# MaartenGr/ReinLife

Hardware: AMD Instinct MI355X
Metric: agent-steps/sec (env.step + policy fwd), 30x30 grid, 100 agents (higher is better)
Workload: dtype f32-grade policy via block-scaled 2 x f16 split on v_mfma_f32_32x32x16_f16 (f32 accumulate) / int32+u8 world state / f64 rewards

## Files before the change

reinlife_amd/csrc/rl_policy_dev.h:

```cpp
#pragma once
#include "rl_common.h"

namespace {

typedef float f32x16 __attribute__((ext_vector_type(16)));
typedef float f32x4 __attribute__((ext_vector_type(4)));
typedef float f32x4u __attribute__((ext_vector_type(4), aligned(4)));
typedef float f32x2 __attribute__((ext_vector_type(2)));
typedef _Float16 f16x8 __attribute__((ext_vector_type(8)));
typedef const float __attribute__((address_space(1))) gfloat;
typedef const f32x4 __attribute__((address_space(1))) gf32x4;

constexpr int kInChunks = 10;
constexpr int kPlanes = 2;
constexpr int kScaleExp = 10;

__host__ __device__ constexpr int64_t frag_floats(int chunks, int tout) { return (int64_t)chunks * tout * kPlanes * 64 * 4; }
__host__ __device__ constexpr int64_t in_layer_floats(int tout) { return frag_floats(kInChunks, tout) + (int64_t)tout * 64; }
__host__ __device__ constexpr int64_t hid_layer_floats(int tin, int tout) { return frag_floats(2 * tin, tout) + (int64_t)tout * 64; }
__host__ __device__ constexpr int64_t head_consts_off(int tin) { return frag_floats(2 * tin, 1); }
__host__ __device__ constexpr int64_t head_floats(int tin, int nout) { return head_consts_off(tin) + 16; }

struct Layout {
    int64_t l1, l2a, l2b, ha, hb, total;
// ... 337 lines not shown
        split8(x, sc0, B1[c][0], B1[c][1]);
    }
    f32x16 acc[4];
    RL_PMARK1(2);
    k_loop_reg4<kInChunks>(w, B1, acc);
    RL_PMARK1(3);
    w.start(packed + L.l2a, lane, 0);
    f32x4 B2[8][kPlanes], B3[8][kPlanes];
    float un1, un2;
    layer_out_to_B(acc, packed + L.l1 + frag_floats(kInChunks, 4), h, un0, B2, un1);
    RL_PMARK1(4);
    k_loop_reg4<8>(w, B2, acc);
    RL_PMARK1(5);
    layer_out_to_B(acc, packed + L.l2a + frag_floats(8, 4), h, un1, B3, un2);
    float adv[4], val[4];
    RL_PMARK1(6);
    head_reg<4>(packed + L.ha, B3, un2, lane, adv);
    RL_PMARK1(7);
    w.start(packed + L.l2b, lane, 0);
    k_loop_reg4<8>(w, B2, acc);
    RL_PMARK1(8);
    layer_out_to_B(acc, packed + L.l2b + frag_floats(8, 4), h, un1, B3, un2);
    head_reg<4>(packed + L.hb, B3, un2, lane, val);
    RL_PMARK1(9);
    const f32x4 ba = ((gf32x4*)(packed + L.ha + head_consts_off(4) + 8))[h];
    tile1_finish<KIND>(io, lane, adv, val[0] + packed[L.hb + head_consts_off(4) + 8], draw, ba);
}

constexpr int kStageUnits = 512;
constexpr int kStages = 10 + 8 + 2 + 8 + 2;
constexpr int kDenseTiles = 4;

constexpr int kTileConstFloats = 3 * 256 + 2 * 16;

template <int NS, int D, int STEPS = 2 * NS, int TOUT = 4>
struct WRingH {
    f32x4 a[D][2][kPlanes];
    gf32x4* p;
#ifdef RL_ABL_WH
    static __host__ __device__ constexpr int off(int i) { return 0; }
#else
    static __host__ __device__ constexpr int off(int i) { return ((i % NS) * TOUT + 2 * (i / NS)) * kPlanes * 64; }
#endif
    __device__ inline void start(gfloat* __restrict__ pw, int lane)
    {
        static_assert(D < NS, "ring deeper than a pass");
        p = (gf32x4*)pw + lane;
#pragma unroll
        for (int d = 0; d < D; ++d)
#pragma unroll
            for (int t = 0; t < 2; ++t)
#pragma unroll
                for (int pl = 0; pl < kPlanes; ++pl) a[d][t][pl] = p[off(d) + (t * kPlanes + pl) * 64];
        p += off(D);
        asm volatile("" : "+v"(p));
    }
    __device__ inline void take(int i, f32x4 (&ac)[2][kPlanes])
    {
        const int cur = i % D;
#pragma unroll
        for (int t = 0; t < 2; ++t)
#pragma unroll
            for (int pl = 0; pl < kPlanes; ++pl) ac[t][pl] = a[cur][t][pl];
        if (i + D < STEPS) {
#pragma unroll
            for (int t = 0; t < 2; ++t)
// ... 126 lines not shown
    f32x16 a0, a1, a2;
#pragma unroll
    for (int r = 0; r < 16; ++r) { a0[r] = 0.0f; a1[r] = 0.0f; a2[r] = 0.0f; }
    f32x4 B[NCH][kPlanes];
#pragma unroll
    for (int k = 0; k < 3; ++k) split_slice<3>(k, [&](int e) { return raw(0, e); }, sc, B[0][0], B[0][1]);
#pragma unroll
    for (int s = 0; s < NCH; ++s) {
        f32x4 ac[1][kPlanes];
        w.template next<NCH>(s, ac);
        a0 = mfma16(ac[0][0], B[s][1], a0);
        if (s + 1 < NCH) split_slice<3>(0, [&](int e) { return raw(s + 1, e); }, sc, B[(s + 1) % NCH][0], B[(s + 1) % NCH][1]);
        __builtin_amdgcn_sched_barrier(0);
        a1 = mfma16(ac[0][0], B[s][0], a1);
        if (s + 1 < NCH) split_slice<3>(1, [&](int e) { return raw(s + 1, e); }, sc, B[(s + 1) % NCH][0], B[(s + 1) % NCH][1]);
        __builtin_amdgcn_sched_barrier(0);
        a2 = mfma16(ac[0][1], B[s][0], a2);
        if (s + 1 < NCH) split_slice<3>(2, [&](int e) { return raw(s + 1, e); }, sc, B[(s + 1) % NCH][0], B[(s + 1) % NCH][1]);
        __builtin_amdgcn_sched_barrier(0);
    }
#pragma unroll
    for (int r = 0; r < 4; ++r) out[r] = ((a0[r] + a1[r]) + a2[r]) * (un4[r] * row_un);
}

struct PairLds {
    float* pmax;
    f32x4* ex;
    float* val;
};
struct Tile1Part {
    float head[4];
    rl_u4 draw;
};
template <int KIND, bool COHERENT, bool PAIR = false, int XM = 0>
__device__ inline void policy_tile1s(const TileIO& io, int lane, int role = 0, const PairLds* pair_lds = nullptr, Tile1Part* part = nullptr)
{
    static_assert(KIND == RL_D3QN || KIND == RL_PERD3QN, "one-wave tile: dueling kinds");
    extern __shared__ __attribute__((aligned(16))) char rl_dyn_lds[];
    constexpr int D = 3;
    const int h = lane >> 5;
    const Layout L = layout_of(KIND);
    gfloat* __restrict__ packed = io.packed;
    const float* const consts = (const float*)(rl_dyn_lds + io.c_lds_off) + 32 * h;
    const float* const hconsts = (const float*)(rl_dyn_lds + io.c_lds_off) + 768;
    RL_PMARK1(1);
    WRingH<kInChunks, D, PAIR ? kInChunks : 2 * kInChunks> w1;
    w1.start(packed + L.l1 + (PAIR ? role * (2 * kPlanes * 64 * 4) : 0), lane);
    f32x4 X[kInChunks][2];
    {
        const int64_t rbase = io.row * RL_OBS_DIM;
        if (io.x_lds_off >= 0) {
            const float* xr = (const float*)(rl_dyn_lds + io.x_lds_off);
#pragma unroll
            for (int c = 0; c < kInChunks; ++c)
#pragma unroll
                for (int q = 0; q < 2; ++q) {
                    if (c == kInChunks - 1 && h == 1) X[c][q] = f32x4{xr[149], xr[150], xr[151], xr[152]};
                    else X[c][q] = *(const f32x4*)(xr + 16 * c + 8 * h + 4 * q);
                }
        } else
#pragma unroll
        for (int c = 0; c < kInChunks; ++c)
#pragma unroll
            for (int q = 0; q < 2; ++q) {
                const int k0 = (c == kInChunks - 1 && h == 1) ? 149 : 16 * c + 8 * h + 4 * q;
                if (COHERENT) {
                    const __amdgpu_buffer_rsrc_t rsrc = __builtin_amdgcn_make_buffer_rsrc((void*)io.obs, 0, 0x7fffffff, 0x00027000);
                    X[c][q] = __builtin_bit_cast(f32x4, __builtin_amdgcn_raw_buffer_load_b128(rsrc, (int)((rbase + k0) * 4), 0, 16 ));
                } else
                    X[c][q] = *(const f32x4u*)(io.obs + rbase + k0);
// ... 15 lines not shown
            }
        float m = fmaxf(fmaxf(m4[0], m4[1]), fmaxf(m4[2], m4[3]));
        m = fmaxf(m, __shfl_xor(m, 32));
        row_scale(m, sc0, un0);
    }
    f32x4 B1[kInChunks][kPlanes];
    auto xraw = [&](int c, int e) { return X[c][e >> 2][e & 3]; };
    f32x16 F[4];
    EpiStream ep;
    if constexpr (XM >= 1) {
        auto x0 = [&](int e) { return xraw(0, e); };
        in_split_slot<XM, 0, 0>(x0, sc0, B1[0][0], B1[0][1]); in_split_slot<XM, 0, 1>(x0, sc0, B1[0][0], B1[0][1]);
        in_split_slot<XM, 0, 2>(x0, sc0, B1[0][0], B1[0][1]); in_split_slot<XM, 0, 3>(x0, sc0, B1[0][0], B1[0][1]);
        RL_PMARK1(2);
        k_pass_inx<0, XM>(w1, B1, F[0], F[1], [&](auto st, auto k, auto) {
            constexpr int c = decltype(st)::value + 1;
            if constexpr (c < kInChunks) in_split_slot<XM, c, decltype(k)::value>([&](int e) { return xraw(c, e); }, sc0, B1[c][0], B1[c][1]);
        });
    } else {
#pragma unroll
        for (int k = 0; k < 6; ++k) split_slice<6>(k, [&](int e) { return xraw(0, e); }, sc0, B1[0][0], B1[0][1]);
        RL_PMARK1(2);
        k_pass<kInChunks, 0>(w1, B1, F[0], F[1], [&](int slot) {
            const int c = slot / 6 + 1;
            if (c < kInChunks) split_slice<6>(slot % 6, [&](int e) { return xraw(c, e); }, sc0, B1[c][0], B1[c][1]);
        });
    }
    float mrow = 0.0f;
    const int64_t l2 = (PAIR && role) ? L.l2b : L.l2a, hd = (PAIR && role) ? L.hb : L.ha;
    WRingH<8, D> w2;
    f32x4 B2[8][kPlanes];
    float sc1, un1;
    auto fraw = [&](int c, int e) { return F[c >> 1][8 * (c & 1) + e]; };
    if (PAIR) {
        w2.start(packed + l2, lane);
        ep.c = consts + role * 128;
        ep.fetch(0, 0);
#pragma unroll
        for (int e = 0; e < 32; ++e) ep.step(0, e, F[0], F[1], un0, mrow);
        mrow = fmaxf(mrow, __shfl_xor(mrow, 32));
        pair_lds->pmax[role * 64 + lane] = mrow;
        lds_barrier();
        mrow = fmaxf(mrow, pair_lds->pmax[(role ^ 1) * 64 + lane]);
        row_scale(mrow, sc1, un1);
#pragma unroll
        for (int c = 0; c < 4; ++c) {
            f32x4 hi, lo;
#pragma unroll
            for (int k = 0; k < 6; ++k) split_slice<6>(k, [&](int e) { return fraw(c, e); }, sc1, hi, lo);
            pair_lds->ex[((4 * role + c) * kPlanes + 0) * 64 + lane] = hi;
            pair_lds->ex[((4 * role + c) * kPlanes + 1) * 64 + lane] = lo;
        }
        lds_barrier();
#pragma unroll
        for (int c = 0; c < 8; ++c)
#pragma unroll
            for (int pl = 0; pl < kPlanes; ++pl) B2[c][pl] = pair_lds->ex[(c * kPlanes + pl) * 64 + lane];
    } else {
        ep.c = consts;
        if constexpr (XM >= 1)
            k_pass_inx<1, XM>(w1, B1, F[2], F[3], [&](auto, auto, auto sl) {
                constexpr int slot = decltype(sl)::value;
                if constexpr (slot == 0) ep.fetch(0, 0);
                if constexpr (slot >= 2 && slot < 34) ep.step(0, slot - 2, F[0], F[1], un0, mrow);
            });
        else
        k_pass<kInChunks, 1>(w1, B1, F[2], F[3], [&](int slot) {
            if (slot == 0) ep.fetch(0, 0);
            if (slot >= 2 && slot < 34) ep.step(0, slot - 2, F[0], F[1], un0, mrow);
        });
        RL_PMARK1(3);
        w2.start(packed + l2, lane);
        ep.fetch(2, 0);
#pragma unroll
        for (int e = 0; e < 32; ++e) ep.step(2, e, F[2], F[3], un0, mrow);
        mrow = fmaxf(mrow, __shfl_xor(mrow, 32));
        row_scale(mrow, sc1, un1);
#pragma unroll
        for (int k = 0; k < 6; ++k) split_slice<6>(k, [&](int e) { return fraw(0, e); }, sc1, B2[0][0], B2[0][1]);
    }
    RL_PMARK1(4);
    f32x16 A[4];
    k_pass<8, 0>(w2, B2, A[0], A[1], [&](int slot) {
        const int c = slot / 6 + 1;
        if (!PAIR && c < 8) split_slice<6>(slot % 6, [&](int e) { return fraw(c, e); }, sc1, B2[c][0], B2[c][1]);
    });
    mrow = 0.0f;
    ep.c = consts + ((PAIR && role) ? 512 : 256);
    k_pass<8, 1>(w2, B2, A[2], A[3], [&](int slot) {
        if (slot == 0) ep.fetch(0, 0);
        if (slot >= 2 && slot < 34) ep.step(0, slot - 2, A[0], A[1], un1, mrow);
    });
    RL_PMARK1(5);
    WRing<1, 1, 1, D> wh;
    wh.start(packed + hd, lane, 0);
    ep.fetch(2, 0);
#pragma unroll
    for (int e = 0; e < 32; ++e) ep.step(2, e, A[2], A[3], un1, mrow);
    mrow = fmaxf(mrow, __shfl_xor(mrow, 32));
    float sc2, un2;
    row_scale(mrow, sc2, un2);
    auto araw = [&](int c, int e) { return A[c >> 1][8 * (c & 1) + e]; };
    float adv[4], val[4];
    RL_PMARK1(6);
    if (PAIR) {
        head_stream<D>(wh, *(const f32x4*)(hconsts + ((PAIR && role) ? 16 : 0) + 4 * h), araw, sc2, un2, adv);
        if (role) { if (h == 0) pair_lds->val[lane] = adv[0] + hconsts[16 + 8]; }
        else {
#pragma unroll
            for (int r = 0; r < 4; ++r) part->head[r] = adv[r];
            part->draw = draw;
        }
        RL_PMARK1(9);
        return;
    }
    head_stream<D>(wh, *(const f32x4*)(hconsts + 4 * h), araw, sc2, un2, adv);
    WRingH<8, D> w3;
    w3.start(packed + L.l2b, lane);
    RL_PMARK1(7);
    k_pass<8, 0>(w3, B2, A[0], A[1], [&](int) {});
    mrow = 0.0f;
    ep.c = consts + 512;
    k_pass<8, 1>(w3, B2, A[2], A[3], [&](int slot) {
        if (slot == 0) ep.fetch(0, 0);
        if (slot >= 2 && slot < 34) ep.step(0, slot - 2, A[0], A[1], un1, mrow);
    });
    RL_PMARK1(8);
    wh.start(packed + L.hb, lane, 0);
    ep.fetch(2, 0);
#pragma unroll
    for (int e = 0; e < 32; ++e) ep.step(2, e, A[2], A[3], un1, mrow);
    mrow = fmaxf(mrow, __shfl_xor(mrow, 32));
    row_scale(mrow, sc2, un2);
    head_stream<D>(wh, *(const f32x4*)(hconsts + 16 + 4 * h), araw, sc2, un2, val);
    RL_PMARK1(9);
    tile1_finish<KIND>(io, lane, adv, val[0] + hconsts[16 + 8], draw, *(const f32x4*)(hconsts + 8 + 4 * h));
}


// ... 809 lines not shown
```

reinlife_amd/csrc/rl_run.hip:

```cpp
#include <mutex>
#include "rl_world_dev.h"
#ifndef RL_XM_DUELING_KERNEL
#define RL_XM_DUELING_KERNEL 0
#endif
#if RL_XM_DUELING_KERNEL != 0 && !defined(RL_XM_SELF_GENERATED_STATES_ONLY)
#error "RL_XM_DUELING_KERNEL != 0 is valid for self-generated states only: add -DRL_XM_SELF_GENERATED_STATES_ONLY to an A/B build that knows"
#endif
#ifndef RL_XM_ALL_DUELING_TILE
#define RL_XM_ALL_DUELING_TILE RL_XM_ALL_KERNEL
#endif
#ifndef RL_XM_ALL_KERNEL
#define RL_XM_ALL_KERNEL 2
#endif

#ifdef RL_TUNING
#if !(defined(RL_RUN_UNIT) && RL_RUN_UNIT == 1)
static int g_run_debug = 0;
extern "C" __attribute__((visibility("default"))) void rl_debug_set_run_mask(int mask) { g_run_debug = mask; }
extern "C" __attribute__((visibility("default"))) int rl_debug_get_run_mask(void) { return g_run_debug; }
#endif
#define RL_RUN_DBG(ka) (*(const int __attribute__((address_space(4)))*)&(ka)->ra.debug)
#else
#define RL_RUN_DBG(ka) 0
#endif

namespace {

#include "rl_policy_dev.h"

constexpr int kRunMaxBrains = 8;
constexpr int kKindAll = 4;
__host__ __device__ constexpr int kind_widest(int KIND) { return KIND == kKindAll ? RL_PPO : KIND; }

#ifndef RL_RUN_COHERENT
#define RL_RUN_COHERENT true
#endif
struct RunArgs {
    const float* packed[kRunMaxBrains];
    float eps[kRunMaxBrains];
    int kind[kRunMaxBrains];
    float* obs[2];
    int first;
    int n_ticks;
    int8_t* actions;
    const float* eps_sched;
    int eps_inline_on;
    float eps_inline[RL_EPS_INLINE_MAX];
    int trk_skip;
    int capture;
    float* policy_out;
    rl_replay rp[kRunMaxBrains];
    int debug;
};

struct PolSmem {
    short* prow;
    int* bstart;
    int* bcnt;
    int* tstart;
    short* trow;
    int* tbrain;
    int* meta;
    float* pairv;
    float* cconst;
    float* xmirror;
    int xrows;
    int xbytes;
    double* trk_scr;
    TrkLds trk;
    int* wtask;
    int* texoff;
    int* bkind;
    int* oflags;
};
constexpr int kMaxTiles = 32;
constexpr int kPairFloats = 32 + 2 * 64;
constexpr int kPairExBytes = 8 * kPlanes * 64 * 16;
constexpr int kPairFloatsAll = kPairValFloats + 2 * 64;
template <int KIND> __host__ __device__ constexpr int run_const_floats() { return KIND == kKindAll ? kTileConstMax : kTileConstFloats; }
template <int KIND> __host__ __device__ constexpr int run_pair_floats() { return KIND == kKindAll ? kPairFloatsAll : kPairFloats; }
template <int KIND>
__host__ __device__ inline size_t carve_policy(PolSmem& ps, char* base, size_t o, int cap, size_t mirror_budget = 0, int n_cbrains = 0,
                                               int pair_floats = run_pair_floats<KIND>(),
                                               size_t min_region = 0)
{
    o = align16(o);
    ps.xmirror = nullptr; ps.xrows = 0; ps.xbytes = 0;
    const size_t tail = 10 * (size_t)cap + 5120 + sizeof(float) * 4 * (size_t)pair_floats + sizeof(float) * run_const_floats<KIND>() * (size_t)n_cbrains;
    if (mirror_budget > o + tail) {
        const size_t rows = (mirror_budget - o - tail) / (sizeof(float) * kXStride);
        ps.xrows = (int)(rows < (size_t)cap ? rows : (size_t)cap);
        if (ps.xrows >= 32) {
            size_t bytes = sizeof(float) * kXStride * (size_t)ps.xrows;
            if (bytes < min_region && o + tail + min_region <= mirror_budget) bytes = min_region;
            ps.xmirror = (float*)(base + o); ps.xbytes = (int)bytes; o = align16(o + bytes);
        } else ps.xrows = 0;
    }
    ps.prow = (short*)(base + o); o = align16(o + sizeof(short) * (size_t)cap);
    ps.bstart = (int*)(base + o); o = align16(o + sizeof(int) * 64);
    ps.bcnt = (int*)(base + o); o = align16(o + sizeof(int) * 64);
    ps.tstart = (int*)(base + o); o = align16(o + sizeof(int) * 64);
    ps.trow = (short*)(base + o); o = align16(o + sizeof(short) * kMaxTiles * 32);
    ps.tbrain = (int*)(base + o); o = align16(o + sizeof(int) * kMaxTiles);
    ps.meta = (int*)(base + o); o = align16(o + sizeof(int) * 16);
    ps.cconst = nullptr;
    if (n_cbrains > 0) { ps.cconst = (float*)(base + o); o = align16(o + sizeof(float) * run_const_floats<KIND>() * (size_t)n_cbrains); }
    ps.pairv = nullptr;
    if (n_cbrains > 0) { ps.pairv = (float*)(base + o); o = align16(o + sizeof(float) * 4 * (size_t)pair_floats); }
    ps.wtask = (int*)(base + o); o = align16(o + sizeof(int) * 8);
    ps.texoff = (int*)(base + o); o = align16(o + sizeof(int) * 4);
    ps.bkind = (int*)(base + o); o = align16(o + sizeof(int) * kRunMaxBrains);
    if (KIND == kKindAll) { ps.oflags = (int*)(base + o); o = align16(o + sizeof(int) * 4); }
// ... 216 lines not shown
        io.prof = (p.prof && (int)blockIdx.x == p.prof_world && wave == 0) ? p.prof : nullptr;
        if (io.prof && lane == 0) { io.prof[100] = t_entry; io.prof[110] = (long long)clock64(); }
#endif
    };
    if constexpr (T == 1024) {
        const int q = __builtin_amdgcn_readfirstlane(wave >> 2), slot = wave & 3;
        for (int t0 = 0; t0 < ntiles; t0 += 4) {
            const int lane = rl_lane_fresh(), j = lane & 31;
            const int ti = t0 + slot;
            const bool have = ti < ntiles;
            TileIO io;
            Tile1Part part;
            QuadLds ql;
            ql.pmax = ps.pairv + kQuadFloats * slot; ql.val = ql.pmax + 3 * 32 * 4;
            ql.ex = (f32x4*)((char*)ps.xmirror + (size_t)kQuadExBytes * slot);
#ifdef RL_PHASE_PROFILE
            ql.prof = (p.prof && (int)blockIdx.x == p.prof_world && slot == 0) ? p.prof : nullptr;
#endif
            if (have) {
                tile_io(ti, io, j);
                if (ntiles > 4) io.x_lds_off = -1;
                policy_quad<KIND, RL_RUN_COHERENT>(io, lane, q, &ql, &part);
            } else {
#pragma unroll
                for (int i = 0; i < kQuadBarriers; ++i) lds_barrier();
            }
            lds_barrier();
            if (have && q == 0) tile1_finish<KIND>(io, lane, part.head, ql.val[j], part.draw, *(const f32x4*)((const float*)(smem_base + io.c_lds_off) + 768 + 8 + 4 * (lane >> 5)));
        }
    } else
    if (T == 512 && ps.pairv != nullptr && ntiles <= 4 && (size_t)ps.xrows * kXStride * sizeof(float) >= 4 * (size_t)kPairExBytes) {
        const int role = __builtin_amdgcn_readfirstlane(wave >> 2), slot = wave & 3;
        const bool have = slot < ntiles;
        TileIO io;
        Tile1Part part;
        PairLds pl;
        pl.val = ps.pairv + kPairFloats * slot; pl.pmax = pl.val + 32;
        pl.ex = (f32x4*)((char*)ps.xmirror + (size_t)kPairExBytes * slot);
        if (have) {
            tile_io(slot, io, j);
            policy_tile1s<KIND, RL_RUN_COHERENT, true, RL_XM_DUELING_KERNEL>(io, lane, role, &pl, &part);
        } else { lds_barrier(); lds_barrier(); }
#ifdef RL_PHASE_PROFILE
        if (p.prof && (int)blockIdx.x == p.prof_world && lane == 0) p.prof[116 + wave] = (long long)clock64();
#endif
        lds_barrier();
        if (have && role == 0) {
            const int fl = rl_lane_fresh();
            tile1_finish<KIND>(io, fl, part.head, pl.val[fl & 31], part.draw, *(const f32x4*)((const float*)(smem_base + io.c_lds_off) + 768 + 8 + 4 * (fl >> 5)));
        }
    } else
    for (int ti = wave; ti < ntiles; ti += T / 64) {
        TileIO io;
        tile_io(ti, io, j);
        if (T == 512) policy_tile1s<KIND, RL_RUN_COHERENT, false, RL_XM_DUELING_KERNEL>(io, lane);
        else policy_tile1<KIND, RL_RUN_COHERENT, true>(io, lane);
    }
#ifdef RL_PHASE_PROFILE
    if (p.prof && (int)blockIdx.x == p.prof_world && tid == 0) p.prof[111] = (long long)clock64();
#endif
    lds_barrier();
#ifdef RL_PHASE_PROFILE
    if (p.prof && (int)blockIdx.x == p.prof_world && tid == 0) p.prof[112] = (long long)clock64();
#endif
}

#ifndef RL_XM_COLD_CALL
#define RL_XM_COLD_CALL 0
#endif
#ifndef RL_XM_LIKELY
#define RL_XM_LIKELY 1
#endif
#if RL_XM_LIKELY
#define RL_XM_EXPECT(x) __builtin_expect_with_probability(!!(x), 1, 0.9)
#else
#define RL_XM_EXPECT(x) (x)
#endif
__device__ __attribute__((noinline, cold)) Tile1Part run_tile_general(TileIO io, PairLds pl, int role, int kind)
{
    Tile1Part part;
    const int lane = rl_lane_fresh();
    if (kind == RL_DQN) policy_pair2<RL_DQN, RL_RUN_COHERENT>(io, lane, role, &pl, &part);
    else if (kind == RL_PPO) policy_pair2<RL_PPO, RL_RUN_COHERENT>(io, lane, role, &pl, &part);
    else policy_tile1s<RL_PERD3QN, RL_RUN_COHERENT, true>(io, lane, role, &pl, &part);
    return part;
}

template <int T, int TRAIN>
__device__ __forceinline__ void run_policy_all(const KParams& p, Smem& s, PolSmem& ps, RunParamsC* ka, int w, int n, const float* obs_rows, char* smem_base, int wave)
{
    static_assert(T == 512, "kKindAll: 512-thread workgroups");
    typedef const int __attribute__((address_space(4))) cint;
    const int lane = rl_lane_fresh(), j = lane & 31;
#ifdef RL_PHASE_PROFILE
    if (p.prof && (int)blockIdx.x == p.prof_world && wave == 0 && lane == 0) p.prof[100] = (long long)clock64();
#endif
    const int ntiles = __builtin_amdgcn_readfirstlane(ps.meta[0]);
    const bool mirrored = ps.xmirror != nullptr && __builtin_amdgcn_readfirstlane(ps.meta[4]) != 0;
    const bool fallback = __builtin_amdgcn_readfirstlane(ps.meta[5]) != 0;
    constexpr int xneed = RL_XM_ALL_KERNEL == 2 ? (RL_XF_SCALE | RL_XF_INT_HEALTH) : RL_XF_SCALE;
#ifdef RL_XM_ASSUME_ALWAYS
    const bool rows_known = true;
#else
    const bool rows_known = RL_XM_ALL_KERNEL != 0 && (__builtin_amdgcn_readfirstlane(ps.oflags[0]) & xneed) == xneed;
#endif
    auto tile_io = [&](int ti, TileIO& io, bool from_mirror, int task) {
        const int b = task >= 0 ? ((task >> 12) & 255) : __builtin_amdgcn_readfirstlane(ps.tbrain[ti]);
        const int e = (unsigned short)ps.trow[ti * 32 + j], k = e & 0x7fff;
        io.packed = (gfloat*)((const float* const __attribute__((address_space(4)))*)ka->ra.packed)[b];
        io.obs = obs_rows;
        io.row = (int64_t)w * p.cap + k;
        io.valid = !(e & 0x8000);
        io.eps = run_eps<TRAIN>(ka, b, p.n_brains, ps);
        io.out = TRAIN == 2 ? *(float* const __attribute__((address_space(4)))*)&ka->ra.policy_out : nullptr;
        io.actions = *(int8_t* const __attribute__((address_space(4)))*)&ka->ra.actions;
        io.seed = p.seed;
        io.key_world = (uint32_t)(p.world_base + w); io.key_tick = (uint32_t)s.scal[S_TICK]; io.key_epoch = (uint32_t)s.scal[S_EPOCH];
        io.key_index = (uint32_t)k;
        io.lds_actions_off = (int)((char*)s.action - smem_base); io.lds_slot = k;
        io.x_lds_off = (from_mirror && mirrored && k < ps.xrows) ? (int)((char*)(ps.xmirror + k * kXStride) - smem_base) : -1;
        io.c_lds_off = (int)((char*)(ps.cconst + kTileConstMax * b) - smem_base);
#ifdef RL_PHASE_PROFILE
        io.prof = (p.prof && (int)blockIdx.x == p.prof_world && wave == ((p.ablate >> 20) & 7)) ? p.prof : nullptr;
#endif
        return task >= 0 ? ((task >> 20) & 7) : ((cint*)ka->ra.kind)[b];
    };
    auto pair_round = [&](bool have, int ti, int role, int slot, int ex_off, bool from_mirror, int task) {
        TileIO io;
        Tile1Part part;
        PairLds pl;
        int kind = -1;
        if (have) {
            kind = __builtin_amdgcn_readfirstlane(tile_io(ti, io, from_mirror, task));
            pl.val = ps.pairv + kPairFloatsAll * slot; pl.pmax = pl.val + kPairValFloats;
            pl.ex = (f32x4*)((char*)ps.xmirror + ex_off);
            const bool plain = kind == RL_DQN || kind == RL_PPO;
            if (!plain && RL_XM_ALL_DUELING_TILE == 0) policy_tile1s<RL_PERD3QN, RL_RUN_COHERENT, true>(io, lane, role, &pl, &part);
            else if (RL_XM_EXPECT(rows_known)) {
                if (kind == RL_DQN) policy_pair2<RL_DQN, RL_RUN_COHERENT, RL_XM_ALL_KERNEL>(io, lane, role, &pl, &part);
                else if (kind == RL_PPO) policy_pair2<RL_PPO, RL_RUN_COHERENT, RL_XM_ALL_KERNEL>(io, lane, role, &pl, &part);
                else policy_tile1s<RL_PERD3QN, RL_RUN_COHERENT, true, RL_XM_ALL_DUELING_TILE>(io, lane, role, &pl, &part);
            } else if (RL_XM_COLD_CALL) part = run_tile_general(io, pl, role, kind);
            else {
                if (kind == RL_DQN) policy_pair2<RL_DQN, RL_RUN_COHERENT>(io, lane, role, &pl, &part);
                else if (kind == RL_PPO) policy_pair2<RL_PPO, RL_RUN_COHERENT>(io, lane, role, &pl, &part);
                else policy_tile1s<RL_PERD3QN, RL_RUN_COHERENT, true>(io, lane, role, &pl, &part);
            }
        } else { lds_barrier(); lds_barrier(); }
        lds_barrier();
        if (have && role == 0) {
            const int fl = rl_lane_fresh();
            if (kind == RL_DQN) pair_finish<RL_DQN>(io, fl, part, &pl);
            else if (kind == RL_PPO) pair_finish<RL_PPO>(io, fl, part, &pl);
            else tile1_finish<RL_PERD3QN>(io, fl, part.head, pl.val[fl & 31], part.draw, *(const f32x4*)((const float*)(smem_base + io.c_lds_off) + 768 + 8 + 4 * (fl >> 5)));
        }
    };
    const int pr = __builtin_amdgcn_readfirstlane(ps.meta[6]);
    const int task = __builtin_amdgcn_readfirstlane(ps.wtask[wave]);
    const int n_rounds = fallback ? (ntiles + pr - 1) / pr : 1;
    for (int r = 0; r < n_rounds; ++r) {
        const int slot = fallback ? (wave & 3) : (task & 255);
        const int ti = fallback ? r * pr + slot : slot;
        const bool have = fallback ? (slot < pr && ti < ntiles) : task >= 0;
        const int role = __builtin_amdgcn_readfirstlane(fallback ? (wave >> 2) : ((task >> 8) & 1));
        const int ex_off = fallback ? slot * pair_ex_bytes(RL_PPO) : (have ? ps.texoff[slot] : 0);
        pair_round(have, ti, role, slot, ex_off, !fallback, fallback ? -1 : task);
        if (fallback) lds_barrier();
    }
#ifdef RL_PHASE_PROFILE
    if (p.prof && (int)blockIdx.x == p.prof_world && lane == 0) p.prof[116 + wave] = (long long)clock64();
    if (p.prof && (int)blockIdx.x == p.prof_world && wave == 0 && lane == 0) p.prof[111] = (long long)clock64();
#endif
    lds_barrier();
#ifdef RL_PHASE_PROFILE
    if (p.prof && (int)blockIdx.x == p.prof_world && wave == 0 && lane == 0) p.prof[112] = (long long)clock64();
#endif
}

template <int T, bool FIXED, int KIND, int TRAIN>
__device__ __forceinline__ void run_policy_half(RunParamsC* ka, int wave)
{
    extern __shared__ __attribute__((aligned(16))) char smem_raw[];
    const KParams p = run_params<FIXED, T>(ka);
    Smem s;
    PolSmem ps;
    run_carve<FIXED, KIND>(p, s, ps, smem_raw, T);
    const int w = blockIdx.x;
// ... 250 lines not shown
    RL_MARK(67);
    if (p.uo.src)
        for (int k = tid; k < n2; k += T) p.uo.src[b + k] = refill ? (short)-1 : s.src[s.order[k]];
    const RecycleRegs rr = recycle_read(s, n2);
    {
        if (tid < 64) {
            policy_lists_wave0(p, ps, n2, tid, [&](int k) { return s.brain[s.order[k]]; });
            if (T == 1024 && tid == 0) ps.meta[5] = ps.meta[0] > 4;
            RL_MARK_T(96, 0);
            if constexpr (KIND == kKindAll) policy_schedule_wave0(p, ps, ka, tid);
            RL_MARK_T(97, 0);
        } else {
            if constexpr (KIND == kKindAll) { if (tid == 64) ps.oflags[0] = run_obs_flags(p, s, n2, ps.oflags[1]); }
            write_observations<(T > 64 ? T - 64 : 64)>(p, s, w, n2, obs_out, tid - 64, ps.xmirror, ps.xrows);
            RL_MARK_T(98, 64); RL_MARK_T(99, T - 64);
        }
    }
    RL_MARK(68);
    if (tid == 0) { ps.meta[1] = n2; ps.meta[2] = cur ^ 1; ps.meta[3] = ticks_done + 1; }
    if (ticks_done == 0 && tid == 0) ps.meta[4] = ps.xmirror != nullptr;
    if (RL_SEAM_OPEN && tid == 64) { s.scal[S_TICK] = tick_next; s.scal[S_EPOCH] = epoch_next; }
    const bool seam_open = RL_SEAM_OPEN && T == 512 && ticks_done + 1 < *(const int __attribute__((address_space(4)))*)&ka->ra.n_ticks;
    recycle_world<T, kSpec>(p, s, n2, tick_next, epoch_next, next_uid, max_gene, ps.xmirror == nullptr || n2 > ps.xrows || (TRAIN == 2 && cap), rr,
                            (KIND == kKindAll || T == 1024) ? &ps.meta[5] : nullptr,
                            seam_open);
    RL_MARK(69);
}

template <int T, int KIND, int TRAIN>
__device__ __forceinline__ void run_tick_call_fixed(RunParamsC* ka) { run_tick_body<T, true, KIND, TRAIN>(ka); }
template <int T, int KIND, int TRAIN>
__device__ __forceinline__ void run_tick_call_generic(RunParamsC* ka) { run_tick_body<T, false, KIND, TRAIN>(ka); }

template <int T, bool FIXED, int KIND, int TRAIN>
__device__ __forceinline__ void run_load_call(RunParamsC* ka)
{
    extern __shared__ __attribute__((aligned(16))) char smem_raw[];
    typedef const int __attribute__((address_space(4))) cint;
    const KParams p = run_params<FIXED, T>(ka);
    Smem s;
    PolSmem ps;
    run_carve<FIXED, KIND>(p, s, ps, smem_raw, T);
    int n0;
    RL_MARK(90);
    const int tid = rl_tidx();
    const int first = *(cint*)&ka->ra.first;
    const int n_pre = ((cint*)ka->p.st.n_agents)[blockIdx.x];
    const bool preload = ps.xmirror != nullptr && n_pre <= ps.xrows;
    constexpr int NT = T > 64 ? T - 64 : T;
    const int pt = T > 64 ? tid - 64 : tid;
    typedef const f32x4 __attribute__((address_space(1))) gvec;
    gvec* rows4 = (gvec*)(((float* const __attribute__((address_space(4)))*)ka->ra.obs)[first] + (size_t)blockIdx.x * p.cap * RL_OBS_DIM);
    const int total = n_pre * RL_OBS_DIM, nvec = (total + 3) >> 2;
    constexpr int U = 8, UC = 4;
    f32x4 rv[U];
    float cv[UC];
    if (preload && pt >= 0 && nvec > 0) {
#pragma unroll
        for (int u = 0; u < U; ++u) rv[u] = rows4[min(u * NT + pt, nvec - 1)];
    }
    constexpr int CF = run_const_floats<KIND>();
    const int ctotal = ps.cconst ? CF * p.n_brains : 0;
    auto const_src = [&](int i) -> gfloat* {
        const int b = i / CF, j = i - CF * b;
        gfloat* pk = (gfloat*)((const float* const __attribute__((address_space(4)))*)ka->ra.packed)[b];
        if constexpr (KIND == kKindAll) {
            const int kind = ((const int __attribute__((address_space(4)))*)ka->ra.kind)[b];
            return pk + tile_const_src(kind, min(j, tile_const_floats(kind) - 1));
        } else
            return pk + tile_const_src(KIND, j);
    };
    if (ctotal > 0) {
#pragma unroll
        for (int u = 0; u < UC; ++u) cv[u] = *const_src(min(u * T + tid, ctotal - 1));
    }
    load_world<T, (T == 1024)>(p, s, (int)blockIdx.x, n0);
    RL_MARK(91);
    auto put_rows = [&](int q, const f32x4& v) {
        if (q < nvec) {
#pragma unroll
            for (int e = 0; e < 4; ++e) {
                const int i = 4 * q + e, r = i / RL_OBS_DIM;
                if (i < total) ps.xmirror[r * kXStride + (i - r * RL_OBS_DIM)] = v[e];
            }
        }
    };
    if (preload && pt >= 0 && nvec > 0) {
#pragma unroll
        for (int u = 0; u < U; ++u) put_rows(u * NT + pt, rv[u]);
        for (int base = NT * U; base < nvec; base += NT * U) {
#pragma unroll
            for (int u = 0; u < U; ++u) rv[u] = rows4[min(base + u * NT + pt, nvec - 1)];
#pragma unroll
            for (int u = 0; u < U; ++u) put_rows(base + u * NT + pt, rv[u]);
        }
    }
    if (preload && pt >= 0)
        for (int r = pt; r < n_pre; r += NT) {
            float* m = ps.xmirror + r * kXStride + 153;
            m[0] = 0.0f; m[1] = 0.0f; m[2] = 0.0f; *(float4*)(m + 3) = float4{0.0f, 0.0f, 0.0f, 0.0f};
        }
    RL_MARK(92);
    if constexpr (KIND == kKindAll) {
// ... 1 lines not shown
        for (int a = tid; a < n0; a += T) bad |= (s.health[a] >= 400 || s.health[a] <= -400) ? 1 : 0;
        bad = __any(bad);
        if (tid == 0) ps.oflags[1] = 0;
        lds_barrier();
        if (bad && (tid & 63) == 0) ps.oflags[1] = 1;
        lds_barrier();
    }
    if (tid == 0) {
        ps.meta[1] = n0; ps.meta[2] = first; ps.meta[3] = 0; ps.meta[4] = preload ? 1 : 0;
        if constexpr (KIND == kKindAll) ps.oflags[0] = run_obs_flags(p, s, n0, ps.oflags[1]);
    }
    if (TRAIN && p.so.trk_tick) {
        const int G = p.static_families ? p.n_brains : 1, t = tid;
        const size_t o = (size_t)blockIdx.x * G * RL_TRK_VARS;
        if (t < G * RL_TRK_VARS) { ps.trk.sum[t] = p.so.trk_sum[o + t]; ps.trk.cnt[t] = p.so.trk_cnt[o + t]; }
        if (t < 2) ps.trk.pop[t] = p.so.trk_pop[(size_t)blockIdx.x * 3 + 1 + t];
    }
    if (tid < 64) {
        if constexpr (KIND == kKindAll) { if (tid < kRunMaxBrains) ps.bkind[tid] = tid < p.n_brains ? ((const int __attribute__((address_space(4)))*)ka->ra.kind)[tid] : RL_D3QN; }
        policy_lists_wave0(p, ps, n0, tid, [&](int k) { return s.brain[k]; });
        if (T == 1024 && tid == 0) ps.meta[5] = ps.meta[0] > 4;
        if constexpr (KIND == kKindAll) policy_schedule_wave0(p, ps, ka, tid, true);
    }
    RL_MARK(93);
    if (ctotal > 0) {
#pragma unroll
        for (int u = 0; u < UC; ++u) { const int i = u * T + tid; if (i < ctotal) ps.cconst[i] = cv[u]; }
        for (int base = T * UC; base < ctotal; base += T * UC) {
#pragma unroll
            for (int u = 0; u < UC; ++u) cv[u] = *const_src(min(base + u * T + tid, ctotal - 1));
#pragma unroll
            for (int u = 0; u < UC; ++u) { const int i = base + u * T + tid; if (i < ctotal) ps.cconst[i] = cv[u]; }
        }
    }
    RL_MARK(94);
    lds_barrier();
    RL_MARK(95);
}
template <int T, bool FIXED, int KIND, int TRAIN>
__device__ __forceinline__ void run_store_call(RunParamsC* ka)
{
    extern __shared__ __attribute__((aligned(16))) char smem_raw[];
    const KParams p = run_params<FIXED, T>(ka);
    Smem s;
    PolSmem ps;
    run_carve<FIXED, KIND>(p, s, ps, smem_raw, T);
    store_world<T>(p, s, (int)blockIdx.x, ps.meta[1]);
    if (TRAIN && p.so.trk_tick) {
        const int G = p.static_families ? p.n_brains : 1, t = rl_tidx();
        const size_t o = (size_t)blockIdx.x * G * RL_TRK_VARS;
        if (t < G * RL_TRK_VARS) { p.so.trk_sum[o + t] = ps.trk.sum[t]; p.so.trk_cnt[o + t] = ps.trk.cnt[t]; }
        if (t < 2) p.so.trk_pop[(size_t)blockIdx.x * 3 + 1 + t] = ps.trk.pop[t];
    }
    if (rl_tidx() == 0) { p.st.tick[blockIdx.x] = s.scal[S_TICK]; p.st.epoch[blockIdx.x] = s.scal[S_EPOCH]; p.st.next_uid[blockIdx.x] = s.scal[S_NEXT_UID]; p.st.max_gene[blockIdx.x] = s.scal[S_MAX_GENE]; }
}

template <int T, bool FIXED, int KIND, int TRAIN>
__global__ __launch_bounds__(T) void k_run(const RunParams rp)
{
    RunParamsC* ka = (RunParamsC*)__builtin_amdgcn_kernarg_segment_ptr();
    typedef const int __attribute__((address_space(4))) cint;
    const int n_ticks = *(cint*)&ka->ra.n_ticks;
    const int dbg = RL_RUN_DBG(ka);
#ifdef RL_PHASE_PROFILE
#define RL_KMARK(i) do { long long* pf_ = *(long long* const __attribute__((address_space(4)))*)&ka->p.prof; \
        if (pf_ && (int)blockIdx.x == *(cint*)&ka->p.prof_world && threadIdx.x == 0) RL_G(pf_)[i] = (long long)clock64(); } while (0)
// ... 200 lines not shown
```

Measured before the change: 1.002 billion.

## Skip value-stream layer via certified argmax bound in dueling pair tile

Adds a certified-argmax path to the paired dueling tile. A per-brain bound on the value stream's magnitude is precomputed at load time from weight norms. When the advantage gap exceeds that bound, the greedy action is fixed without computing the value stream, so the second wave exits early and skips its hidden layer, head and final barrier. Rows that cannot be certified fall back to a cold noinline full computation, which adds bound computation at load, extra constants, and possible divergence.

```diff
diff --git a/reinlife_amd/csrc/rl_policy_dev.h b/reinlife_amd/csrc/rl_policy_dev.h
--- a/reinlife_amd/csrc/rl_policy_dev.h
+++ b/reinlife_amd/csrc/rl_policy_dev.h
@@ -393,6 +393,7 @@
 constexpr int kDenseTiles = 4;
 
 constexpr int kTileConstFloats = 3 * 256 + 2 * 16;
+constexpr int kTileCertFloats = 4;
 
 template <int NS, int D, int STEPS = 2 * NS, int TOUT = 4>
 struct WRingH {
@@ -585,10 +586,131 @@
     float head[4];
     rl_u4 draw;
 };
-template <int KIND, bool COHERENT, bool PAIR = false, int XM = 0>
+
+#ifndef RL_CERT_COUNT
+#define RL_CERT_COUNT(greedy_mask, cert_mask, fell_back) do { } while (0)
+#endif
+template <int KIND>
+__device__ __attribute__((noinline, cold)) void tile1_cert_fallback(TileIO io, const f32x4* ex, float un1, f32x4 adv4, rl_u4 draw)
+{
+    extern __shared__ __attribute__((aligned(16))) char rl_dyn_lds[];
+    constexpr int D = 3;
+    const int lane = (int)__builtin_amdgcn_mbcnt_hi(~0u, __builtin_amdgcn_mbcnt_lo(~0u, 0u)), h = lane >> 5;
+    const Layout L = layout_of(KIND);
+    const float* const consts = (const float*)(rl_dyn_lds + io.c_lds_off) + 32 * h;
+    const float* const hconsts = (const float*)(rl_dyn_lds + io.c_lds_off) + 768;
+    WRingH<8, D> w;
+    w.start(io.packed + L.l2b, lane);
+    f32x4 B2[8][kPlanes];
+#pragma unroll
+    for (int c = 0; c < 8; ++c)
+#pragma unroll
+        for (int pl = 0; pl < kPlanes; ++pl) B2[c][pl] = ex[(c * kPlanes + pl) * 64 + lane];
+    f32x16 A[4];
+    EpiStream ep;
+    float mrow = 0.0f;
+    k_pass<8, 0>(w, B2, A[0], A[1], [&](int) {});
+    ep.c = consts + 512;
+    k_pass<8, 1>(w, B2, A[2], A[3], [&](int slot) {
+        if (slot == 0) ep.fetch(0, 0);
+        if (slot >= 2 && slot < 34) ep.step(0, slot - 2, A[0], A[1], un1, mrow);
+    });
+    WRing<1, 1, 1, D> wh;
+    wh.start(io.packed + L.hb, lane, 0);
+    ep.fetch(2, 0);
+#pragma unroll
+    for (int e = 0; e < 32; ++e) ep.step(2, e, A[2], A[3], un1, mrow);
+    mrow = fmaxf(mrow, __shfl_xor(mrow, 32));
+    float sc2, un2;
+    row_scale(mrow, sc2, un2);
+    auto araw = [&](int c, int e) { return A[c >> 1][8 * (c & 1) + e]; };
+    float val[4];
+    head_stream<D>(wh, *(const f32x4*)(hconsts + 16 + 4 * h), araw, sc2, un2, val);
+    const float adv[4] = {adv4.x, adv4.y, adv4.z, adv4.w};
+    tile1_finish<KIND>(io, lane, adv, val[0] + hconsts[16 + 8], draw, *(const f32x4*)(hconsts + 8 + 4 * h));
+}
+template <int KIND>
+__device__ inline void tile1_finish_cert(const TileIO& io, int lane, const float (&adv)[4], const rl_u4& draw, const float* hconsts, float vbar,
+                                         const f32x4* ex, float un1)
+{
+    const int h = lane >> 5;
+    const f32x4 ba = *(const f32x4*)(hconsts + 8 + 4 * h);
+    const float a4[4] = {adv[0] + ba.x, adv[1] + ba.y, adv[2] + ba.z, adv[3] + ba.w};
+    float o4[4];
+#pragma unroll
+    for (int r = 0; r < 4; ++r) o4[r] = __shfl_xor(a4[r], 32);
+    int act = 0;
+    bool greedy = false, ok = true;
+    if (h == 0) {
+        const float a[8] = {a4[0], a4[1], a4[2], a4[3], o4[0], o4[1], o4[2], o4[3]};
+        float best = a[0], amax = fabsf(a[0]), s = a[0];
+        int is = 0;
+#pragma unroll
+        for (int i = 1; i < 8; ++i) {
+            const bool gt = a[i] > best;
+            is = gt ? i : is; best = gt ? a[i] : best;
+            amax = fmaxf(amax, fabsf(a[i])); s += a[i];
+        }
+        const float thr = 0x1p-20f * (((amax + amax) + vbar) + 0x1p-80f) + (s - s);
+#pragma unroll
+        for (int j = 0; j < 7; ++j) ok = ok && (j >= is || best - a[j] > thr);
+        const bool explore = (float)rl_u24(draw.x) < io.eps;
+        act = explore ? (int)(draw.y >> 29) : is;
+        greedy = io.valid && io.actions && !explore;
+    }
+    const bool need = greedy && !ok;
+    RL_CERT_COUNT(__ballot(greedy), __ballot(greedy && ok), __any(need));
+    if (__builtin_expect(__any(need), 0)) {
+        tile1_cert_fallback<KIND>(io, ex, un1, f32x4{adv[0], adv[1], adv[2], adv[3]}, draw);
+        return;
+    }
+    if (h == 0 && io.valid && io.actions) {
+        io.actions[io.row] = (int8_t)act;
+        if (io.lds_actions_off >= 0) {
+            extern __shared__ __attribute__((aligned(16))) char rl_dyn_lds[];
+            ((signed char*)rl_dyn_lds)[io.lds_actions_off + io.lds_slot] = (signed char)act;
+        }
+    }
+}
+
+__device__ inline void cert_bound_part(gfloat* __restrict__ pk, int tid, double& c0, double& c1)
+{
+    const Layout L = layout_of(RL_PERD3QN);
+    const int t2 = tid >> 7, pl = (tid >> 6) & 1, lane = tid & 63, oo = lane & 31, o = 32 * t2 + oo;
+    const int h = (oo >> 2) & 1, r = (oo & 3) + 4 * (oo >> 3);
+    gf32x4* f = (gf32x4*)(pk + L.l2b) + (t2 * kPlanes + pl) * 64 + lane;
+    f32x4 u[8];
+#pragma unroll
+    for (int s = 0; s < 8; ++s) u[s] = f[s * 4 * kPlanes * 64];
+    const float un_o = pk[L.l2b + frag_floats(8, 4) + (t2 * 2 + h) * 32 + r], b1 = pk[L.l2b + frag_floats(8, 4) + (t2 * 2 + h) * 32 + 16 + r];
+    typedef const _Float16 __attribute__((address_space(1))) gf16;
+    gf16* hw = (gf16*)(pk + L.hb);
+    const int hidx = (((o >> 5) * 2 + (r >> 3)) * kPlanes * 64 + 32 * h) * 8 + (r & 7);
+    const double w = (double)fabsf((float)hw[hidx]) + (double)fabsf((float)hw[hidx + 64 * 8]);
+    const double un_v = (double)pk[L.hb + head_consts_off(4)];
+    double sum = 0.0;
+#pragma unroll
+    for (int s = 0; s < 8; ++s) {
+        const f16x8 v = __builtin_bit_cast(f16x8, u[s]);
+#pragma unroll
+        for (int e = 0; e < 8; ++e) sum += (double)fabsf((float)v[e]);
+    }
+    const double wv = w * un_v;
+    c1 = wv * (sum * (double)un_o);
+    c0 = (pl == 0 && lane < 32) ? wv * (double)fabsf(b1) : 0.0;
+}
+__device__ inline float f32_up(double d)
+{
+    float f = (float)d;
+    if ((double)f < d) f = __builtin_bit_cast(float, __builtin_bit_cast(unsigned, f) + (f >= 0.0f ? 1u : -1u));
+    return f;
+}
+
+template <int KIND, bool COHERENT, bool PAIR = false, int XM = 0, bool CERT = false>
 __device__ inline void policy_tile1s(const TileIO& io, int lane, int role = 0, const PairLds* pair_lds = nullptr, Tile1Part* part = nullptr)
 {
     static_assert(KIND == RL_D3QN || KIND == RL_PERD3QN, "one-wave tile: dueling kinds");
+    static_assert(!CERT || PAIR, "the certified argmax: the pair tile");
     extern __shared__ __attribute__((aligned(16))) char rl_dyn_lds[];
     constexpr int D = 3;
     const int h = lane >> 5;
@@ -670,8 +792,9 @@
     f32x4 B2[8][kPlanes];
     float sc1, un1;
     auto fraw = [&](int c, int e) { return F[c >> 1][8 * (c & 1) + e]; };
+    [[maybe_unused]] float zrow = 0.0f;
     if (PAIR) {
-        w2.start(packed + l2, lane);
+        if (!(CERT && role)) w2.start(packed + l2, lane);
         ep.c = consts + role * 128;
         ep.fetch(0, 0);
 #pragma unroll
@@ -680,6 +803,7 @@
         pair_lds->pmax[role * 64 + lane] = mrow;
         lds_barrier();
         mrow = fmaxf(mrow, pair_lds->pmax[(role ^ 1) * 64 + lane]);
+        zrow = mrow;
         row_scale(mrow, sc1, un1);
 #pragma unroll
         for (int c = 0; c < 4; ++c) {
@@ -690,6 +814,7 @@
             pair_lds->ex[((4 * role + c) * kPlanes + 1) * 64 + lane] = lo;
         }
         lds_barrier();
+        if (CERT && role) { RL_PMARK1(9); return; }
 #pragma unroll
         for (int c = 0; c < 8; ++c)
 #pragma unroll
@@ -743,6 +868,12 @@
     RL_PMARK1(6);
     if (PAIR) {
         head_stream<D>(wh, *(const f32x4*)(hconsts + ((PAIR && role) ? 16 : 0) + 4 * h), araw, sc2, un2, adv);
+        if constexpr (CERT) {
+            const float* const kc = hconsts + kTileConstFloats - 768;
+            tile1_finish_cert<KIND>(io, lane, adv, draw, hconsts, __builtin_fmaf(kc[1], zrow, kc[0]), pair_lds->ex, un1);
+            RL_PMARK1(9);
+            return;
+        }
         if (role) { if (h == 0) pair_lds->val[lane] = adv[0] + hconsts[16 + 8]; }
         else {
 #pragma unroll
diff --git a/reinlife_amd/csrc/rl_run.hip b/reinlife_amd/csrc/rl_run.hip
--- a/reinlife_amd/csrc/rl_run.hip
+++ b/reinlife_amd/csrc/rl_run.hip
@@ -8,6 +8,9 @@
 #endif
 #ifndef RL_XM_ALL_DUELING_TILE
 #define RL_XM_ALL_DUELING_TILE RL_XM_ALL_KERNEL
+#endif
+#ifndef RL_CERT_ALL
+#define RL_CERT_ALL 0
 #endif
 #ifndef RL_XM_ALL_KERNEL
 #define RL_XM_ALL_KERNEL 2
@@ -20,8 +23,26 @@
 extern "C" __attribute__((visibility("default"))) int rl_debug_get_run_mask(void) { return g_run_debug; }
 #endif
 #define RL_RUN_DBG(ka) (*(const int __attribute__((address_space(4)))*)&(ka)->ra.debug)
+static __device__ unsigned long long g_cert_counts[4];
+#define RL_CERT_COUNT(greedy_mask, cert_mask, fell_back) do { \
+        const unsigned long long gm_ = (greedy_mask), cm_ = (cert_mask); const bool fb_ = (fell_back); \
+        if (__builtin_amdgcn_mbcnt_hi(~0u, __builtin_amdgcn_mbcnt_lo(~0u, 0u)) == 0) { \
+            atomicAdd(&g_cert_counts[0], (unsigned long long)__popcll(gm_)); atomicAdd(&g_cert_counts[1], (unsigned long long)__popcll(cm_)); \
+            if (fb_) atomicAdd(&g_cert_counts[2], 1ull); } } while (0)
 #else
 #define RL_RUN_DBG(ka) 0
+#endif
+#ifdef RL_TUNING
+#if defined(RL_RUN_UNIT) && RL_RUN_UNIT == 1
+extern "C" __attribute__((visibility("default"))) int rl_debug_cert_counters_all(unsigned long long* out)
+#else
+extern "C" __attribute__((visibility("default"))) int rl_debug_cert_counters(unsigned long long* out)
+#endif
+{
+    const unsigned long long zero[4] = {0, 0, 0, 0};
+    if (hipDeviceSynchronize() != hipSuccess || hipMemcpyFromSymbol(out, HIP_SYMBOL(g_cert_counts), sizeof(zero)) != hipSuccess) return -1;
+    return hipMemcpyToSymbol(HIP_SYMBOL(g_cert_counts), zero, sizeof(zero)) == hipSuccess ? 0 : -1;
+}
 #endif
 
 namespace {
@@ -77,7 +98,8 @@
 constexpr int kPairFloats = 32 + 2 * 64;
 constexpr int kPairExBytes = 8 * kPlanes * 64 * 16;
 constexpr int kPairFloatsAll = kPairValFloats + 2 * 64;
-template <int KIND> __host__ __device__ constexpr int run_const_floats() { return KIND == kKindAll ? kTileConstMax : kTileConstFloats; }
+template <int KIND> __host__ __device__ constexpr int run_const_floats() { return KIND == kKindAll ? kTileConstMax : kTileConstFloats + kTileCertFloats; }
+static_assert(kTileConstFloats + kTileCertFloats <= kTileConstMax, "kKindAll: the dueling block's value bound fits behind its constants");
 template <int KIND> __host__ __device__ constexpr int run_pair_floats() { return KIND == kKindAll ? kPairFloatsAll : kPairFloats; }
 template <int KIND>
 __host__ __device__ inline size_t carve_policy(PolSmem& ps, char* base, size_t o, int cap, size_t mirror_budget = 0, int n_cbrains = 0,
@@ -360,6 +382,7 @@
     if (T == 512 && ps.pairv != nullptr && ntiles <= 4 && (size_t)ps.xrows * kXStride * sizeof(float) >= 4 * (size_t)kPairExBytes) {
         const int role = __builtin_amdgcn_readfirstlane(wave >> 2), slot = wave & 3;
         const bool have = slot < ntiles;
+        const bool cert = TRAIN != 2 && !(RL_RUN_DBG(ka) & 64);
         TileIO io;
         Tile1Part part;
         PairLds pl;
@@ -367,15 +390,18 @@
         pl.ex = (f32x4*)((char*)ps.xmirror + (size_t)kPairExBytes * slot);
         if (have) {
             tile_io(slot, io, j);
-            policy_tile1s<KIND, RL_RUN_COHERENT, true, RL_XM_DUELING_KERNEL>(io, lane, role, &pl, &part);
+            if (cert) policy_tile1s<KIND, RL_RUN_COHERENT, true, RL_XM_DUELING_KERNEL, TRAIN != 2>(io, lane, role, &pl, &part);
+            else policy_tile1s<KIND, RL_RUN_COHERENT, true, RL_XM_DUELING_KERNEL>(io, lane, role, &pl, &part);
         } else { lds_barrier(); lds_barrier(); }
 #ifdef RL_PHASE_PROFILE
         if (p.prof && (int)blockIdx.x == p.prof_world && lane == 0) p.prof[116 + wave] = (long long)clock64();
 #endif
-        lds_barrier();
-        if (have && role == 0) {
-            const int fl = rl_lane_fresh();
-            tile1_finish<KIND>(io, fl, part.head, pl.val[fl & 31], part.draw, *(const f32x4*)((const float*)(smem_base + io.c_lds_off) + 768 + 8 + 4 * (fl >> 5)));
+        if (!cert) {
+            lds_barrier();
+            if (have && role == 0) {
+                const int fl = rl_lane_fresh();
+                tile1_finish<KIND>(io, fl, part.head, pl.val[fl & 31], part.draw, *(const f32x4*)((const float*)(smem_base + io.c_lds_off) + 768 + 8 + 4 * (fl >> 5)));
+            }
         }
     } else
     for (int ti = wave; ti < ntiles; ti += T / 64) {
@@ -404,13 +430,14 @@
 #else
 #define RL_XM_EXPECT(x) (x)
 #endif
+template <bool CERT>
 __device__ __attribute__((noinline, cold)) Tile1Part run_tile_general(TileIO io, PairLds pl, int role, int kind)
 {
     Tile1Part part;
     const int lane = rl_lane_fresh();
     if (kind == RL_DQN) policy_pair2<RL_DQN, RL_RUN_COHERENT>(io, lane, role, &pl, &part);
     else if (kind == RL_PPO) policy_pair2<RL_PPO, RL_RUN_COHERENT>(io, lane, role, &pl, &part);
-    else policy_tile1s<RL_PERD3QN, RL_RUN_COHERENT, true>(io, lane, role, &pl, &part);
+    else policy_tile1s<RL_PERD3QN, RL_RUN_COHERENT, true, 0, CERT>(io, lane, role, &pl, &part);
     return part;
 }
 
@@ -453,6 +480,11 @@
 #endif
         return task >= 0 ? ((task >> 20) & 7) : ((cint*)ka->ra.kind)[b];
     };
+    const bool cert = RL_CERT_ALL && TRAIN != 2 && !(RL_RUN_DBG(ka) & 64);
+    auto duel = [&](auto xm, TileIO& io, int role, PairLds& pl, Tile1Part& part) {
+        if (cert) policy_tile1s<RL_PERD3QN, RL_RUN_COHERENT, true, decltype(xm)::value, TRAIN != 2>(io, lane, role, &pl, &part);
+        else policy_tile1s<RL_PERD3QN, RL_RUN_COHERENT, true, decltype(xm)::value>(io, lane, role, &pl, &part);
+    };
     auto pair_round = [&](bool have, int ti, int role, int slot, int ex_off, bool from_mirror, int task) {
         TileIO io;
         Tile1Part part;
@@ -463,16 +495,16 @@
             pl.val = ps.pairv + kPairFloatsAll * slot; pl.pmax = pl.val + kPairValFloats;
             pl.ex = (f32x4*)((char*)ps.xmirror + ex_off);
             const bool plain = kind == RL_DQN || kind == RL_PPO;
-            if (!plain && RL_XM_ALL_DUELING_TILE == 0) policy_tile1s<RL_PERD3QN, RL_RUN_COHERENT, true>(io, lane, role, &pl, &part);
+            if (!plain && RL_XM_ALL_DUELING_TILE == 0) duel(IntC<0>{}, io, role, pl, part);
             else if (RL_XM_EXPECT(rows_known)) {
                 if (kind == RL_DQN) policy_pair2<RL_DQN, RL_RUN_COHERENT, RL_XM_ALL_KERNEL>(io, lane, role, &pl, &part);
                 else if (kind == RL_PPO) policy_pair2<RL_PPO, RL_RUN_COHERENT, RL_XM_ALL_KERNEL>(io, lane, role, &pl, &part);
-                else policy_tile1s<RL_PERD3QN, RL_RUN_COHERENT, true, RL_XM_ALL_DUELING_TILE>(io, lane, role, &pl, &part);
-            } else if (RL_XM_COLD_CALL) part = run_tile_general(io, pl, role, kind);
+                else duel(IntC<RL_XM_ALL_DUELING_TILE>{}, io, role, pl, part);
+            } else if (RL_XM_COLD_CALL) part = cert ? run_tile_general<TRAIN != 2>(io, pl, role, kind) : run_tile_general<false>(io, pl, role, kind);
             else {
                 if (kind == RL_DQN) policy_pair2<RL_DQN, RL_RUN_COHERENT>(io, lane, role, &pl, &part);
                 else if (kind == RL_PPO) policy_pair2<RL_PPO, RL_RUN_COHERENT>(io, lane, role, &pl, &part);
-                else policy_tile1s<RL_PERD3QN, RL_RUN_COHERENT, true>(io, lane, role, &pl, &part);
+                else duel(IntC<0>{}, io, role, pl, part);
             }
         } else { lds_barrier(); lds_barrier(); }
         lds_barrier();
@@ -480,7 +512,7 @@
             const int fl = rl_lane_fresh();
             if (kind == RL_DQN) pair_finish<RL_DQN>(io, fl, part, &pl);
             else if (kind == RL_PPO) pair_finish<RL_PPO>(io, fl, part, &pl);
-            else tile1_finish<RL_PERD3QN>(io, fl, part.head, pl.val[fl & 31], part.draw, *(const f32x4*)((const float*)(smem_base + io.c_lds_off) + 768 + 8 + 4 * (fl >> 5)));
+            else if (!cert) tile1_finish<RL_PERD3QN>(io, fl, part.head, pl.val[fl & 31], part.draw, *(const f32x4*)((const float*)(smem_base + io.c_lds_off) + 768 + 8 + 4 * (fl >> 5)));
         }
     };
     const int pr = __builtin_amdgcn_readfirstlane(ps.meta[6]);
@@ -797,6 +829,42 @@
 template <int T, int KIND, int TRAIN>
 __device__ __forceinline__ void run_tick_call_generic(RunParamsC* ka) { run_tick_body<T, false, KIND, TRAIN>(ka); }
 
+template <int KIND>
+__device__ inline void run_cert_bounds(const KParams& p, PolSmem& ps, RunParamsC* ka, int tid)
+{
+    typedef const int __attribute__((address_space(4))) cint;
+    constexpr int CF = run_const_floats<KIND>();
+    const int nb = p.n_brains, wave = tid >> 6;
+    auto dueling = [&](int b) { return KIND != kKindAll || ((cint*)ka->ra.kind)[b] == RL_D3QN || ((cint*)ka->ra.kind)[b] == RL_PERD3QN; };
+    double* part = (double*)ps.pairv;
+    for (int b0 = 0; b0 < nb; b0 += 2) {
+        double c[2][2];
+#pragma unroll
+        for (int i = 0; i < 2; ++i) {
+            const int b = b0 + i;
+            c[i][0] = 0.0; c[i][1] = 0.0;
+            if (b < nb && dueling(b)) cert_bound_part((gfloat*)((const float* const __attribute__((address_space(4)))*)ka->ra.packed)[b], tid, c[i][0], c[i][1]);
+        }
+#pragma unroll
+        for (int off = 32; off >= 1; off >>= 1)
+#pragma unroll
+            for (int i = 0; i < 2; ++i) { c[i][0] += __shfl_xor(c[i][0], off); c[i][1] += __shfl_xor(c[i][1], off); }
+        if ((tid & 63) == 0) {
+#pragma unroll
+            for (int i = 0; i < 2; ++i)
+                if (b0 + i < nb) { part[((b0 + i) * 8 + wave) * 2] = c[i][0]; part[((b0 + i) * 8 + wave) * 2 + 1] = c[i][1]; }
+        }
+    }
+    lds_barrier();
+    if (tid < nb && dueling(tid)) {
+        double c0 = 0.0, c1 = 0.0;
+        for (int w = 0; w < 8; ++w) { c0 += part[(tid * 8 + w) * 2]; c1 += part[(tid * 8 + w) * 2 + 1]; }
+        float* const k = ps.cconst + CF * tid;
+        k[kTileConstFloats] = f32_up(((double)fabsf(k[768 + 16 + 8]) + c0) * (1.0 + 0x1p-8));
+        k[kTileConstFloats + 1] = f32_up(c1 * (1.0 + 0x1p-8));
+    }
+}
+
 template <int T, bool FIXED, int KIND, int TRAIN>
 __device__ __forceinline__ void run_load_call(RunParamsC* ka)
 {
@@ -833,7 +901,7 @@
             const int kind = ((const int __attribute__((address_space(4)))*)ka->ra.kind)[b];
             return pk + tile_const_src(kind, min(j, tile_const_floats(kind) - 1));
         } else
-            return pk + tile_const_src(KIND, j);
+            return pk + tile_const_src(KIND, min(j, kTileConstFloats - 1));
     };
     if (ctotal > 0) {
 #pragma unroll
@@ -901,6 +969,7 @@
 #pragma unroll
             for (int u = 0; u < UC; ++u) { const int i = base + u * T + tid; if (i < ctotal) ps.cconst[i] = cv[u]; }
         }
+        if constexpr (T == 512 && (KIND != kKindAll || RL_CERT_ALL)) run_cert_bounds<KIND>(p, ps, ka, tid);
     }
     RL_MARK(94);
     lds_barrier();
```

Measured after the change: 1.079 billion, median of 6. 1.08x the previous value.
